# Coder-Yu/QRec

Measured on NVIDIA H100. Metric: BPR triples/sec at d=64, higher is better.
Workload: dtype f32

## Files before the change

### qrec_b200/csrc/bpr_kernels.cu

```cuda
#include <cmath>

#include "common.h"
#include "device.cuh"
#include "philox.cuh"
#include "bpr_step.cuh"

namespace {

using namespace qrec;
using namespace qrec::bpr;

template <typename T, int E>
__global__ void __launch_bounds__(256)
bpr_sgd_ordered_kernel(T* __restrict__ P, T* __restrict__ Q, int d, long long n,
                       const int* __restrict__ u, const int* __restrict__ i,
                       const int* __restrict__ j, const int* __restrict__ wu,
                       const int* __restrict__ wi, const int* __restrict__ wj, int* ver_p,
                       int* ver_q, unsigned long long* ticket, T lr, T reg_u, T reg_i,
                       double* loss) {
  const int lane = threadIdx.x & 31;
  double local_loss = 0.0;
  const T a_u = mul_rn(lr, reg_u), a_i = mul_rn(lr, reg_i);
  while (true) {
    unsigned long long k = 0;
    if (lane == 0) k = atomicAdd(ticket, 1ULL);
    k = __shfl_sync(0xffffffffu, k, 0);
    if (k >= (unsigned long long)n) break;
    const int uu = u[k], ii = i[k], jj = j[k];
    const int* vp = lane == 0 ? ver_p + uu : (lane == 1 ? ver_q + ii : ver_q + jj);
    const int need = lane == 0 ? wu[k] : (lane == 1 ? wi[k] : wj[k]);
    unsigned backoff = 8, polls = 0;
    while (true) {
      const int have = lane < 3 ? ld_acquire_gpu(vp) : need;
      if (__all_sync(0xffffffffu, have == need)) break;
      __nanosleep(backoff);
      if (backoff < 64) backoff <<= 1;
      if (++polls > (1u << 27)) __trap();
    }
    T* pr = P + (size_t)uu * d;
    T* qir = Q + (size_t)ii * d;
    T* qjr = Q + (size_t)jj * d;
    T p[E], qi[E], qj[E];
    T di = 0, dj = 0;
#pragma unroll
    for (int e = 0; e < E; ++e) {
      const int c = e * 32 + lane;
      if (c < d) {
        p[e] = __ldcg(pr + c);
        qi[e] = __ldcg(qir + c);
        qj[e] = __ldcg(qjr + c);
        di += p[e] * qi[e];
        dj += p[e] * qj[e];
      } else {
        p[e] = qi[e] = qj[e] = 0;
      }
    }
    di = warp_sum(di);
    dj = warp_sum(dj);
// ... 187 lines not shown
          p[r] = *reinterpret_cast<const float4*>(P + (size_t)uu[r] * D + l * 4);
          qi[r] = *reinterpret_cast<const float4*>(Q + (size_t)ii[r] * D + l * 4);
          qj[r] = *reinterpret_cast<const float4*>(Q + (size_t)jj[r] * D + l * 4);
        } else {
          p[r] = qi[r] = qj[r] = make_float4(0.f, 0.f, 0.f, 0.f);
        }
      }
      if (l < 3) asm volatile("cp.async.bulk.wait_group.read 1;" ::: "memory");
      __syncwarp();
      float* slot = my_stage + (size_t)buf * SLOT_FLOATS;
#pragma unroll
      for (int r = 0; r < UNROLL; ++r) {
        float x = dot4(p[r], qi[r]) - dot4(p[r], qj[r]);
        x = group_sum<LPR>(x);
        const float s = fast_sigmoid(x);
        const float g = lr * (1.0f - s);
        if (ok[r]) {
          if (l == 0) lsum += fast_neg_log(s);
          float4 dp, dqi, dqj;
          bpr_step4(p[r], qi[r], qj[r], g, a_u, a_i, dp, dqi, dqj);
          float* trip = slot + (size_t)(r * TPW + sub) * ROWS * D;
          if (TMA_MASK & 1) *reinterpret_cast<float4*>(trip + SLOT_P * D + l * 4) = dp;
          else red_add_v4(P + (size_t)uu[r] * D + l * 4, dp);
          if (TMA_MASK & 2) *reinterpret_cast<float4*>(trip + SLOT_I * D + l * 4) = dqi;
          else red_add_v4(Q + (size_t)ii[r] * D + l * 4, dqi);
          if (TMA_MASK & 4) *reinterpret_cast<float4*>(trip + SLOT_J * D + l * 4) = dqj;
          else red_add_v4(Q + (size_t)jj[r] * D + l * 4, dqj);
        }
      }
      asm volatile("fence.proxy.async.shared::cta;" ::: "memory");
      __syncwarp();
      if (l < 3 && ((TMA_MASK >> l) & 1)) {
        const int srow = (l == 0) ? SLOT_P : (l == 1 ? SLOT_I : SLOT_J);
#pragma unroll
        for (int r = 0; r < UNROLL; ++r) {
          if (ok[r]) {
            float* dst = (l == 0) ? (P + (size_t)uu[r] * D) : (Q + (size_t)(l == 1 ? ii[r] : jj[r]) * D);
            const float* src = slot + (size_t)(r * TPW + sub) * ROWS * D + srow * D;
            asm volatile("cp.reduce.async.bulk.global.shared::cta.bulk_group.add.f32 [%0], [%1], %2;" ::"l"(dst),
                         "r"((uint32_t)__cvta_generic_to_shared(src)), "n"(D * 4)
                         : "memory");
          }
        }
        asm volatile("cp.async.bulk.commit_group;" ::: "memory");
      }
      buf ^= 1;
    }
  }
  if (l < 3) asm volatile("cp.async.bulk.wait_group 0;" ::: "memory");
  block_add_loss(lsum, loss);
}


constexpr int UM_CH = 32;
constexpr int UM_STAGE_FLOATS = 2 * 4 * 64;
constexpr int UM_STAGE_GROUPS = 16;
constexpr int UM_STAGE_SMEM = UM_STAGE_GROUPS * 2 * (UM_STAGE_FLOATS * 4 + 8);

__device__ __forceinline__ void bulk_row_load(float* smem_dst, const float* gsrc, uint64_t* bar) {
  asm volatile("cp.async.bulk.shared::cluster.global.mbarrier::complete_tx::bytes [%0], [%1], 256, [%2];"
               ::"r"(smem_u32(smem_dst)), "l"(gsrc), "r"(smem_u32(bar)) : "memory");
}

template <int LPR, int G, int CH, bool FULL, bool SAMPLE, bool SIG, bool TMA>
__device__ __forceinline__ void
usermajor_epoch(float* __restrict__ P, float* __restrict__ Q, const float* __restrict__ Qr, int nvec, int n_users,
                long long n, long long ch_begin, long long ch_end, const long long* __restrict__ rowptr,
                const int* __restrict__ i, const int* __restrict__ j, float lr,
                float reg_u, float reg_i, double* loss, FusedSampler fs, long long trip_off,
                const uint32_t* __restrict__ rated_sig) {
  static_assert(!TMA || (LPR == 16 && G == 4 && FULL), "the TMA fetch is laid out for d = 64, G = 4");
  constexpr int GPW = 32 / LPR;
  const int lane = threadIdx.x & 31;
  const int sub = lane / LPR, l = lane % LPR;
  const unsigned gmask = (LPR == 32) ? 0xffffffffu : (((1u << LPR) - 1u) << (sub * LPR));
  const long long group = (((long long)blockIdx.x * blockDim.x + threadIdx.x) >> 5) * GPW + sub;
  const long long ngroups = (((long long)gridDim.x * blockDim.x) >> 5) * GPW;
  const int d = FULL ? LPR * 4 : nvec * 4;
  const bool act = FULL ? true : (l < nvec);
  const float a_u = lr * reg_u, a_i = lr * reg_i;
  const float one_m_au = 1.0f - a_u, one_m_ai = 1.0f - a_i;
  float lsum = 0.f;
  float* stage = nullptr;
  uint64_t* bar = nullptr;
  uint32_t phase0 = 0, phase1 = 0;
  if constexpr (TMA) {
    extern __shared__ __align__(128) unsigned char smem_raw[];
    float* stage_all = reinterpret_cast<float*>(smem_raw);
    uint64_t* bars = reinterpret_cast<uint64_t*>(stage_all + UM_STAGE_GROUPS * 2 * UM_STAGE_FLOATS);
    const int g_in_cta = (threadIdx.x >> 5) * GPW + sub;
    stage = stage_all + (size_t)g_in_cta * 2 * UM_STAGE_FLOATS;
    bar = bars + g_in_cta * 2;
    if (l == 0) { mbar_init(bar, 1); mbar_init(bar + 1, 1); }
    asm volatile("fence.mbarrier_init.release.cluster;" ::: "memory");
    asm volatile("fence.proxy.async.shared::cta;" ::: "memory");
    __syncthreads();
  }
  auto user_of = [&](long long t) {
    int a = 0, b = n_users - 1;
    while (a < b) {
      const int len = b - a + 1;
      const int step = (len + LPR - 1) / LPR;
      int pp = a + (l + 1) * step - 1;
      if (pp > b) pp = b;
      const bool pred = (__ldg(rowptr + pp + 1) - trip_off) > t;
      const unsigned bal = (__ballot_sync(gmask, pred) & gmask) >> (sub * LPR);
      const int f = __ffs(bal) - 1;
      int pf = a + (f + 1) * step - 1;
      if (pf > b) pf = b;
      a = a + f * step;
      b = pf;
    }
    return a;
  };
  for (long long ch = ch_begin + group; ch < ch_end; ch += ngroups) {
    long long lo = ch * CH;
    long long hi = (lo + CH) < n ? (lo + CH) : n;
    int uu = user_of(lo);
    if (lo > 0 && __ldg(rowptr + uu) - trip_off < lo) {
      lo = __ldg(rowptr + uu + 1) - trip_off;
      ++uu;
    }
    if (hi < n) {
      const int ub = user_of(hi);
      if (__ldg(rowptr + ub) - trip_off < hi) {
        const long long e = __ldg(rowptr + ub + 1) - trip_off;
        hi = e < n ? e : n;
      }
    }
    if (lo >= hi) continue;
    long long uend = __ldg(rowptr + uu + 1) - trip_off;
    float* prow = P + (size_t)uu * d + l * 4;
    float4 p = act ? *reinterpret_cast<const float4*>(prow) : make_float4(0.f, 0.f, 0.f, 0.f);
    float4 p0 = p;
    for (long long base = lo; base < hi; base += LPR) {
      const int m = (hi - base) < LPR ? (int)(hi - base) : LPR;
      int mi = 0, mj = 0;
      if (l < m) {
        mi = __ldg(i + base + l);
        if (SAMPLE) {
          int us = uu;
          long long ue = uend;
          while (ue <= base + l) {
            ++us;
            ue = __ldg(rowptr + us + 1) - trip_off;
          }
          if (SIG)
            mj = qrec::sample_negative_sig(base + l + trip_off, fs.epoch, fs.seed_lo, fs.seed_hi, fs.num_items,
                                           fs.rated_cols, __ldg(fs.rated_rowptr + us), __ldg(fs.rated_rowptr + us + 1),
                                           rated_sig + (size_t)us * qrec::RATED_SIG_WORDS);
          else
            mj = qrec::sample_negative(base + l + trip_off, fs.epoch, fs.seed_lo, fs.seed_hi, fs.num_items, fs.rated_cols,
                                       __ldg(fs.rated_rowptr + us), __ldg(fs.rated_rowptr + us + 1));
          if (fs.j_out != nullptr) fs.j_out[base + l] = mj;
        } else {
          mj = __ldg(j + base + l);
        }
      }
      auto issue = [&](int t0) {
        const int src = sub * LPR + ((t0 + (l >> 1)) & (LPR - 1));
        const int idi = __shfl_sync(gmask, mi, src), idj = __shfl_sync(gmask, mj, src);
        const int rows_now = 2 * ((m - t0) < G ? (m - t0) : G);
        uint64_t* bb = bar + ((t0 / G) & 1);
        if (l == 0) mbar_expect_tx(bb, 256u * rows_now);
        __syncwarp(gmask);
        if (l < rows_now) bulk_row_load(stage + ((t0 / G) & 1) * UM_STAGE_FLOATS + l * 64, Qr + (size_t)((l & 1) ? idj : idi) * d, bb);
      };
      if constexpr (TMA) issue(0);
      for (int t0 = 0; t0 < m; t0 += G) {
        const float* slot = nullptr;
        if constexpr (TMA) {
          if (t0 + G < m) issue(t0 + G);
          const int s = (t0 / G) & 1;
          mbar_wait(bar + s, s ? phase1 : phase0);
          if (s) phase1 ^= 1u; else phase0 ^= 1u;
          slot = stage + s * UM_STAGE_FLOATS;
        }
        float4 qi[G], qj[G];
        int ri[G], rj[G];
#pragma unroll
        for (int f = 0; f < G; ++f) {
          ri[f] = __shfl_sync(gmask, mi, sub * LPR + ((t0 + f) & (LPR - 1)));
          rj[f] = __shfl_sync(gmask, mj, sub * LPR + ((t0 + f) & (LPR - 1)));
          if (t0 + f < m && act) {
            if constexpr (TMA) {
              qi[f] = *reinterpret_cast<const float4*>(slot + (2 * f) * 64 + l * 4);
              qj[f] = *reinterpret_cast<const float4*>(slot + (2 * f + 1) * 64 + l * 4);
            } else {
              qi[f] = __ldg(reinterpret_cast<const float4*>(Qr + (size_t)ri[f] * d + l * 4));
              qj[f] = __ldg(reinterpret_cast<const float4*>(Qr + (size_t)rj[f] * d + l * 4));
            }
          } else {
            qi[f] = qj[f] = make_float4(0.f, 0.f, 0.f, 0.f);
          }
        }
        if constexpr (TMA) __syncwarp(gmask);
#pragma unroll
        for (int f = 0; f < G; ++f) {
          const long long t = base + t0 + f;
          if (t0 + f < m) {
            if (t >= uend) {
              if (act) red_add_v4(prow, make_float4(p.x - p0.x, p.y - p0.y, p.z - p0.z, p.w - p0.w));
              do {
                ++uu;
                uend = __ldg(rowptr + uu + 1) - trip_off;
              } while (uend <= t);
              prow = P + (size_t)uu * d + l * 4;
              p = act ? *reinterpret_cast<const float4*>(prow) : make_float4(0.f, 0.f, 0.f, 0.f);
              p0 = p;
            }
            float x = dot4(p, qi[f]) - dot4(p, qj[f]);
            x = group_sum<LPR>(x, gmask);
            const float s = fast_sigmoid(x);
            const float g = lr * (1.0f - s);
            if (l == 0) lsum += fast_neg_log(s);
            if (act) {
              float4 dqi, dqj;
              bpr_step4_inplace(p, qi[f], qj[f], g, one_m_au, g * one_m_ai, a_i, dqi, dqj);
              red_add_v4(Q + (size_t)ri[f] * d + l * 4, dqi);
              red_add_v4(Q + (size_t)rj[f] * d + l * 4, dqj);
            }
          }
        }
      }
    }
    if (act) red_add_v4(prow, make_float4(p.x - p0.x, p.y - p0.y, p.z - p0.z, p.w - p0.w));
  }
  block_add_loss(lsum, loss);
}

template <int LPR, int G, int CH, bool FULL, bool SAMPLE, int MINB = 3, bool SIG = false>
__global__ void __launch_bounds__(256, MINB)
bpr_sgd_usermajor_kernel(float* __restrict__ P, float* __restrict__ Q, const float* __restrict__ Qr, int nvec, int n_users,
                         long long n, long long ch_begin, long long ch_end, const long long* __restrict__ rowptr,
                         const int* __restrict__ i, const int* __restrict__ j, float lr,
                         float reg_u, float reg_i, double* loss, FusedSampler fs, long long trip_off,
                         const uint32_t* __restrict__ rated_sig) {
  usermajor_epoch<LPR, G, CH, FULL, SAMPLE, SIG, false>(P, Q, Qr, nvec, n_users, n, ch_begin, ch_end, rowptr, i, j, lr,
                                                         reg_u, reg_i, loss, fs, trip_off, rated_sig);
}

__global__ void __launch_bounds__(256, 3)
bpr_sgd_usermajor_tma_kernel(float* __restrict__ P, float* __restrict__ Q, const float* __restrict__ Qr, int nvec,
                             int n_users, long long n, long long ch_begin, long long ch_end,
                             const long long* __restrict__ rowptr, const int* __restrict__ i, const int* __restrict__ j,
                             float lr, float reg_u, float reg_i, double* loss, FusedSampler fs, long long trip_off,
                             const uint32_t* __restrict__ rated_sig) {
  usermajor_epoch<16, 4, UM_CH, true, true, false, true>(P, Q, Qr, nvec, n_users, n, ch_begin, ch_end, rowptr, i, j,
                                                         lr, reg_u, reg_i, loss, fs, trip_off, rated_sig);
}

using UserMajorKernel = decltype(&bpr_sgd_usermajor_tma_kernel);

template <int LPR>
UserMajorKernel usermajor_kernel(int nvec, bool sample, bool sig) {
  if (nvec != LPR)
    return sample ? bpr_sgd_usermajor_kernel<LPR, 4, UM_CH, false, true> : bpr_sgd_usermajor_kernel<LPR, 4, UM_CH, false, false>;
  if (sig) return bpr_sgd_usermajor_kernel<LPR, 4, UM_CH, true, true, 3, true>;
  return sample ? bpr_sgd_usermajor_kernel<LPR, 4, UM_CH, true, true> : bpr_sgd_usermajor_kernel<LPR, 4, UM_CH, true, false>;
}

__global__ void __launch_bounds__(256)
rated_signature_kernel(int n_users, const long long* __restrict__ rowptr, const int* __restrict__ cols,
                       uint32_t* __restrict__ sig) {
  const int lane = threadIdx.x & 31;
  const long long warp = ((long long)blockIdx.x * blockDim.x + threadIdx.x) >> 5;
  const long long nwarps = ((long long)gridDim.x * blockDim.x) >> 5;
  for (long long uu = warp; uu < n_users; uu += nwarps) {
    const long long lo = __ldg(rowptr + uu), hi = __ldg(rowptr + uu + 1);
    for (long long e = lo + lane; e < hi; e += 32) {
      const int c = __ldg(cols + e);
      atomicOr(sig + (size_t)uu * qrec::RATED_SIG_WORDS + ((c >> 5) & (qrec::RATED_SIG_WORDS - 1)), 1u << (c & 31));
    }
  }
}

template <typename T>
__global__ void __launch_bounds__(256)
sumsq_kernel(const T* __restrict__ x, long long n, double* out) {
  double acc = 0.0;
  const long long tid = (long long)blockIdx.x * blockDim.x + threadIdx.x;
  const long long stride = (long long)gridDim.x * blockDim.x;
  if constexpr (sizeof(T) == 4) {
    const long long n4 = n >> 2;
    const float4* x4 = reinterpret_cast<const float4*>(x);
    for (long long k = tid; k < n4; k += stride) {
      const float4 v = __ldg(x4 + k);
      acc += (double)v.x * v.x + (double)v.y * v.y + (double)v.z * v.z + (double)v.w * v.w;
    }
    for (long long k = (n4 << 2) + tid; k < n; k += stride) acc += (double)x[k] * x[k];
  } else {
    for (long long k = tid; k < n; k += stride) acc += (double)x[k] * (double)x[k];
  }
  acc = warp_sum(acc);
  __shared__ double wsum[8];
  if ((threadIdx.x & 31) == 0) wsum[threadIdx.x >> 5] = acc;
  __syncthreads();
  if (threadIdx.x == 0) {
    double t = 0.0;
    for (int w = 0; w < (int)(blockDim.x >> 5); ++w) t += wsum[w];
    atomicAdd(out, t);
  }
}

template <typename T>
int launch_ordered(T* P, T* Q, int d, long long n, const int* u, const int* i, const int* j,
                   const int* wu, const int* wi, const int* wj, int* ver_p, int* ver_q,
                   unsigned long long* ticket, T lr, T reg_u, T reg_i, double* loss,
                   int n_warps, cudaStream_t st) {
  QREC_REQUIRE(P && Q && loss && ticket && ver_p && ver_q, "bpr_sgd_ordered: null pointer");
  QREC_REQUIRE(d >= 1 && d <= 256, "bpr_sgd_ordered: d=%d unsupported (1..256)", d);
  QREC_REQUIRE(n >= 0, "bpr_sgd_ordered: n < 0");
// ... 59 lines not shown
                             double reg_u, double reg_i, double* loss, int32_t n_warps, void* stream) {
  return launch_ordered<double>(P, Q, d, n, u, i, j, wu, wi, wj, ver_p, ver_q, ticket, lr, reg_u,
                                reg_i, loss, n_warps, (cudaStream_t)stream);
}

int qrec_bpr_sgd_batch_f32(float* P, float* Q, int32_t d, int64_t n, const int32_t* u,
                           const int32_t* i, const int32_t* j, float lr, float reg_u,
                           float reg_i, double* loss, void* stream) {
  return qrec::launch_bpr_batch(P, Q, d, n, u, i, j, lr, reg_u, reg_i, loss, (cudaStream_t)stream);
}

int qrec_bpr_sgd_batch_tma_f32(float* P, float* Q, int32_t d, int64_t n, const int32_t* u,
                               const int32_t* i, const int32_t* j, float lr, float reg_u,
                               float reg_i, double* loss, void* stream) {
  QREC_REQUIRE(P && Q && loss, "qrec_bpr_sgd_batch_tma_f32: null pointer");
  QREC_REQUIRE(d == 64, "qrec_bpr_sgd_batch_tma_f32: only d=64 (got %d); use qrec_bpr_sgd_batch_f32", d);
  QREC_REQUIRE(n >= 0, "qrec_bpr_sgd_batch_tma_f32: n < 0");
  if (n == 0) return QREC_OK;
  QREC_REQUIRE(u && i && j, "qrec_bpr_sgd_batch_tma_f32: null index pointer");
  constexpr int UN = 4, MASK = 1;
  constexpr int smem = 8 * 2 * UN * 2 * 64 * 4;
  QREC_CUDA(allow_dynamic_smem((const void*)bpr_sgd_batch_tma_kernel<UN, MASK>, smem));
  const int grid = capped_grid(((n + 31) / 32 + 7) / 8, 2);
  bpr_sgd_batch_tma_kernel<UN, MASK><<<grid, 256, smem, (cudaStream_t)stream>>>(P, Q, n, u, i, j, lr, reg_u, reg_i, loss);
  QREC_LAUNCH_CHECK();
  return QREC_OK;
}

}

namespace qrec {
int launch_usermajor(float* P, float* Q, int32_t d, int32_t n_users, int64_t n, const int64_t* rowptr,
                     const int32_t* i, const int32_t* j, float lr, float reg_u, float reg_i, double* loss,
                     bool sample, const int64_t* rated_rowptr, const int32_t* rated_cols, int32_t num_items,
                     uint64_t seed, uint32_t epoch, int32_t* j_out, long long trip_off, cudaStream_t st,
                     const uint32_t* rated_sig, bool tma) {
  if (n <= 0) return QREC_OK;
  QREC_REQUIRE(num_items >= 1, "qrec user-major epoch: num_items=%d (the item table's rows) must be given", num_items);
  QREC_REQUIRE(!tma || (d == 64 && sample), "qrec user-major epoch: the TMA fetch needs d = 64 and fused sampling");
  FusedSampler fs = {reinterpret_cast<const long long*>(rated_rowptr), rated_cols, num_items, (uint32_t)seed,
                     (uint32_t)(seed >> 32), epoch, j_out};
  const int nvec = d / 4;
  const int lpr = nvec <= 4 ? 4 : nvec <= 8 ? 8 : nvec <= 16 ? 16 : 32;
  const bool sig = sample && rated_sig != nullptr;
  const UserMajorKernel kernel = tma        ? bpr_sgd_usermajor_tma_kernel
                                 : lpr == 4  ? usermajor_kernel<4>(nvec, sample, sig)
                                 : lpr == 8  ? usermajor_kernel<8>(nvec, sample, sig)
                                 : lpr == 16 ? usermajor_kernel<16>(nvec, sample, sig)
                                             : usermajor_kernel<32>(nvec, sample, sig);
  const int smem = tma ? UM_STAGE_SMEM : 0;
  if (tma) QREC_CUDA(allow_dynamic_smem((const void*)kernel, smem));
  int occ = 3;
  if (cudaOccupancyMaxActiveBlocksPerMultiprocessor(&occ, kernel, 256, smem) != cudaSuccess || occ < 1) occ = 3;
  const long long nchunks = (n + UM_CH - 1) / UM_CH;
  const long long per_block = 8 * (32 / lpr);
  const int grid = capped_grid((nchunks + per_block - 1) / per_block, occ);
  const size_t q_bytes = (size_t)num_items * d * sizeof(float);
  const long long copy_bytes = 2 * (long long)q_bytes;
  const long long copy_floor = copy_bytes > (8LL << 20) ? 8 * copy_bytes / (24LL * d + 12) : 0;
  long long wave_triples = n / 64 > copy_floor ? n / 64 : copy_floor;
  if (wave_triples > 4LL * num_items) wave_triples = 4LL * num_items;
  const long long wave = wave_triples / UM_CH > 1 ? wave_triples / UM_CH : 1;
  float* Qr = nullptr;
  QREC_CUDA(cudaMallocAsync(reinterpret_cast<void**>(&Qr), q_bytes, st));
  const int rc = [&]() -> int {
    for (long long c0 = 0; c0 < nchunks; c0 += wave) {
      QREC_CUDA(cudaMemcpyAsync(Qr, Q, q_bytes, cudaMemcpyDeviceToDevice, st));
      const long long c1 = (c0 + wave) < nchunks ? (c0 + wave) : nchunks;
      kernel<<<grid, 256, smem, st>>>(P, Q, Qr, nvec, n_users, n, c0, c1, reinterpret_cast<const long long*>(rowptr), i, j,
                                      lr, reg_u, reg_i, loss, fs, trip_off, rated_sig);
      QREC_CUDA(cudaGetLastError());
      if (c1 < nchunks) count_launch();
    }
    return QREC_OK;
  }();
  QREC_CUDA(cudaFreeAsync(Qr, st));
  if (rc != QREC_OK) return rc;
  QREC_LAUNCH_CHECK();
  return QREC_OK;
}
}

extern "C" {

int qrec_bpr_sgd_usermajor_f32(float* P, float* Q, int32_t d, int32_t n_users, int64_t n, int32_t num_items,
                               const int64_t* rowptr, const int32_t* i, const int32_t* j, float lr, float reg_u, float reg_i,
                               double* loss, void* stream) {
  QREC_REQUIRE(P && Q && loss, "qrec_bpr_sgd_usermajor_f32: null pointer");
  QREC_REQUIRE(d >= 4 && d <= 128 && (d % 4) == 0, "qrec_bpr_sgd_usermajor_f32: d=%d unsupported (multiple of 4, 4..128)", d);
  QREC_REQUIRE(n_users >= 0 && n >= 0, "qrec_bpr_sgd_usermajor_f32: negative size");
  if (n_users == 0 || n == 0) return QREC_OK;
  QREC_REQUIRE(rowptr && i && j, "qrec_bpr_sgd_usermajor_f32: null index pointer");
  return qrec::launch_usermajor(P, Q, d, n_users, n, rowptr, i, j, lr, reg_u, reg_i, loss, false, nullptr, nullptr, num_items,
                                0, 0, nullptr, 0, (cudaStream_t)stream, nullptr, false);
}

int qrec_bpr_epoch_usermajor_f32(float* P, float* Q, int32_t d, int32_t n_users, int64_t n, const int64_t* rowptr,
                                 const int32_t* i, const int64_t* rated_rowptr, const int32_t* rated_cols,
                                 int32_t num_items, uint64_t seed, uint32_t epoch, int32_t* j_out, float lr,
                                 float reg_u, float reg_i, double* loss, void* stream) {
  QREC_REQUIRE(P && Q && loss, "qrec_bpr_epoch_usermajor_f32: null pointer");
  QREC_REQUIRE(d >= 4 && d <= 128 && (d % 4) == 0, "qrec_bpr_epoch_usermajor_f32: d=%d unsupported (multiple of 4, 4..128)", d);
  QREC_REQUIRE(n_users >= 0 && n >= 0 && num_items >= 1, "qrec_bpr_epoch_usermajor_f32: bad size");
  if (n_users == 0 || n == 0) return QREC_OK;
  QREC_REQUIRE(rowptr && i && rated_rowptr && rated_cols, "qrec_bpr_epoch_usermajor_f32: null index pointer");
  return qrec::launch_usermajor(P, Q, d, n_users, n, rowptr, i, nullptr, lr, reg_u, reg_i, loss, true, rated_rowptr,
                                rated_cols, num_items, seed, epoch, j_out, 0, (cudaStream_t)stream, nullptr, false);
}

int qrec_rated_signature_build(int32_t n_users, const int64_t* rated_rowptr, const int32_t* rated_cols,
                               uint32_t* sig, void* stream) {
  QREC_REQUIRE(n_users >= 0, "qrec_rated_signature_build: n_users < 0");
  if (n_users == 0) return QREC_OK;
  QREC_REQUIRE(rated_rowptr && rated_cols && sig, "qrec_rated_signature_build: null pointer");
  cudaStream_t st = (cudaStream_t)stream;
  QREC_CUDA(cudaMemsetAsync(sig, 0, (size_t)n_users * qrec::RATED_SIG_WORDS * sizeof(uint32_t), st));
  rated_signature_kernel<<<capped_grid(((long long)n_users + 7) / 8, 8), 256, 0, st>>>(n_users, reinterpret_cast<const long long*>(rated_rowptr),
                                                     rated_cols, sig);
  QREC_LAUNCH_CHECK();
  return QREC_OK;
}

int qrec_bpr_epoch_usermajor_sig_f32(float* P, float* Q, int32_t d, int32_t n_users, int64_t n, const int64_t* rowptr,
                                     const int32_t* i, const int64_t* rated_rowptr, const int32_t* rated_cols,
                                     const uint32_t* rated_sig, int32_t num_items, uint64_t seed, uint32_t epoch,
                                     int32_t* j_out, float lr, float reg_u, float reg_i, double* loss, void* stream) {
  QREC_REQUIRE(P && Q && loss, "qrec_bpr_epoch_usermajor_sig_f32: null pointer");
  QREC_REQUIRE(d == 16 || d == 32 || d == 64 || d == 128,
// ... 67 lines not shown
```

### qrec_b200/csrc/philox.cuh

```cuda
#pragma once
#include <cstdint>

namespace qrec {

__device__ __forceinline__ void philox4x32_10(uint32_t c0, uint32_t c1, uint32_t c2, uint32_t c3,
                                              uint32_t k0, uint32_t k1, uint32_t out[4]) {
  constexpr uint32_t M0 = 0xD2511F53u, M1 = 0xCD9E8D57u, W0 = 0x9E3779B9u, W1 = 0xBB67AE85u;
#pragma unroll
  for (int r = 0; r < 10; ++r) {
    const uint32_t hi0 = __umulhi(M0, c0), lo0 = M0 * c0;
    const uint32_t hi1 = __umulhi(M1, c2), lo1 = M1 * c2;
    const uint32_t n0 = hi1 ^ c1 ^ k0, n1 = lo1, n2 = hi0 ^ c3 ^ k1, n3 = lo0;
    c0 = n0; c1 = n1; c2 = n2; c3 = n3;
    k0 += W0; k1 += W1;
  }
  out[0] = c0; out[1] = c1; out[2] = c2; out[3] = c3;
}

__device__ __forceinline__ int sample_negative(long long k, uint32_t epoch, uint32_t seed_lo, uint32_t seed_hi,
                                               int num_items, const int* __restrict__ cols, long long lo0,
                                               long long hi0) {
  const bool saturated = (hi0 - lo0) >= (long long)num_items;
  uint32_t attempt = 0;
  while (true) {
    uint32_t w[4];
    philox4x32_10((uint32_t)k, (uint32_t)((unsigned long long)k >> 32), attempt, epoch, seed_lo, seed_hi, w);
    const int j = (int)(((unsigned long long)w[0] * (unsigned long long)(uint32_t)num_items) >> 32);
    if (saturated) return j;
    long long lo = lo0, hi = hi0;
    bool hit = false;
    while (lo < hi) {
      const long long mid = (lo + hi) >> 1;
      const int c = __ldg(cols + mid);
      if (c < j) lo = mid + 1;
      else if (c > j) hi = mid;
      else { hit = true; break; }
    }
    if (!hit) return j;
    ++attempt;
  }
}

constexpr int RATED_SIG_WORDS = 16;
__device__ __forceinline__ int sample_negative_sig(long long k, uint32_t epoch, uint32_t seed_lo, uint32_t seed_hi,
                                                   int num_items, const int* __restrict__ cols, long long lo0,
                                                   long long hi0, const uint32_t* __restrict__ sig) {
  const bool saturated = (hi0 - lo0) >= (long long)num_items;
  uint32_t attempt = 0;
  while (true) {
    uint32_t w[4];
    philox4x32_10((uint32_t)k, (uint32_t)((unsigned long long)k >> 32), attempt, epoch, seed_lo, seed_hi, w);
    const int j = (int)(((unsigned long long)w[0] * (unsigned long long)(uint32_t)num_items) >> 32);
    if (saturated) return j;
    const uint32_t word = __ldg(sig + ((j >> 5) & (RATED_SIG_WORDS - 1)));
    if (((word >> (j & 31)) & 1u) == 0u) return j;
    long long lo = lo0, hi = hi0;
    bool hit = false;
    while (lo < hi) {
      const long long mid = (lo + hi) >> 1;
      const int c = __ldg(cols + mid);
      if (c < j) lo = mid + 1;
      else if (c > j) hi = mid;
      else { hit = true; break; }
    }
    if (!hit) return j;
    ++attempt;
  }
}

struct FusedSampler {
  const long long* rated_rowptr;
  const int* rated_cols;
  int num_items;
  uint32_t seed_lo, seed_hi, epoch;
  int* j_out;
};

}
```

Measured before the change: 2.650 billion.

## Schedule user-major BPR by precomputed per-wave user plan with register-cached rated lists

Replaces chunk-based scheduling (per-chunk warp-cooperative binary search over rowptr plus mid-chunk user switching) with a small plan kernel that binary-searches wave boundaries once. Each group then processes whole users strided across the grid. Per-user rated-item lists (up to 64) and signature words are cached in registers, and negative-sample rejection is done by warp shuffles instead of per-lane global binary search. This cuts index-search and scattered-load overhead, but load balance now depends on user-degree skew, and the all-to-all shuffle check costs many instructions.

After: 2.692 billion, median of 6. +1.6%, better.

```diff
diff --git a/qrec_b200/csrc/bpr_kernels.cu b/qrec_b200/csrc/bpr_kernels.cu
--- a/qrec_b200/csrc/bpr_kernels.cu
+++ b/qrec_b200/csrc/bpr_kernels.cu
@@ -298,6 +298,7 @@
 
 
 constexpr int UM_CH = 32;
+constexpr int UM_RATED_PER_LANE = 4;
 constexpr int UM_STAGE_FLOATS = 2 * 4 * 64;
 constexpr int UM_STAGE_GROUPS = 16;
 constexpr int UM_STAGE_SMEM = UM_STAGE_GROUPS * 2 * (UM_STAGE_FLOATS * 4 + 8);
@@ -307,10 +308,27 @@
                ::"r"(smem_u32(smem_dst)), "l"(gsrc), "r"(smem_u32(bar)) : "memory");
 }
 
-template <int LPR, int G, int CH, bool FULL, bool SAMPLE, bool SIG, bool TMA>
+__global__ void __launch_bounds__(256)
+usermajor_wave_plan_kernel(const long long* __restrict__ rowptr, int n_users, long long trip_off, long long wave_triples,
+                           int n_waves, int* __restrict__ plan) {
+  const int w = blockIdx.x * blockDim.x + threadIdx.x;
+  if (w > n_waves) return;
+  if (w == n_waves) { plan[w] = n_users; return; }
+  const long long t = (long long)w * wave_triples;
+  int a = 0, b = n_users;
+  while (a < b) {
+    const int mid = (a + b) >> 1;
+    const long long s = __ldg(rowptr + mid) - trip_off;
+    if ((s > 0 ? s : 0) >= t) b = mid;
+    else a = mid + 1;
+  }
+  plan[w] = a;
+}
+
+template <int LPR, int G, bool FULL, bool SAMPLE, bool SIG, bool TMA>
 __device__ __forceinline__ void
-usermajor_epoch(float* __restrict__ P, float* __restrict__ Q, const float* __restrict__ Qr, int nvec, int n_users,
-                long long n, long long ch_begin, long long ch_end, const long long* __restrict__ rowptr,
+usermajor_epoch(float* __restrict__ P, float* __restrict__ Q, const float* __restrict__ Qr, int nvec, long long n,
+                const int* __restrict__ plan, int wave, const long long* __restrict__ rowptr,
                 const int* __restrict__ i, const int* __restrict__ j, float lr,
                 float reg_u, float reg_i, double* loss, FusedSampler fs, long long trip_off,
                 const uint32_t* __restrict__ rated_sig) {
@@ -319,8 +337,8 @@
   const int lane = threadIdx.x & 31;
   const int sub = lane / LPR, l = lane % LPR;
   const unsigned gmask = (LPR == 32) ? 0xffffffffu : (((1u << LPR) - 1u) << (sub * LPR));
-  const long long group = (((long long)blockIdx.x * blockDim.x + threadIdx.x) >> 5) * GPW + sub;
-  const long long ngroups = (((long long)gridDim.x * blockDim.x) >> 5) * GPW;
+  const int g_in_cta = (threadIdx.x >> 5) * GPW + sub;
+  const int ngroups = gridDim.x * (int)(blockDim.x / LPR);
   const int d = FULL ? LPR * 4 : nvec * 4;
   const bool act = FULL ? true : (l < nvec);
   const float a_u = lr * reg_u, a_i = lr * reg_i;
@@ -333,7 +351,6 @@
     extern __shared__ __align__(128) unsigned char smem_raw[];
     float* stage_all = reinterpret_cast<float*>(smem_raw);
     uint64_t* bars = reinterpret_cast<uint64_t*>(stage_all + UM_STAGE_GROUPS * 2 * UM_STAGE_FLOATS);
-    const int g_in_cta = (threadIdx.x >> 5) * GPW + sub;
     stage = stage_all + (size_t)g_in_cta * 2 * UM_STAGE_FLOATS;
     bar = bars + g_in_cta * 2;
     if (l == 0) { mbar_init(bar, 1); mbar_init(bar + 1, 1); }
@@ -341,66 +358,72 @@
     asm volatile("fence.proxy.async.shared::cta;" ::: "memory");
     __syncthreads();
   }
-  auto user_of = [&](long long t) {
-    int a = 0, b = n_users - 1;
-    while (a < b) {
-      const int len = b - a + 1;
-      const int step = (len + LPR - 1) / LPR;
-      int pp = a + (l + 1) * step - 1;
-      if (pp > b) pp = b;
-      const bool pred = (__ldg(rowptr + pp + 1) - trip_off) > t;
-      const unsigned bal = (__ballot_sync(gmask, pred) & gmask) >> (sub * LPR);
-      const int f = __ffs(bal) - 1;
-      int pf = a + (f + 1) * step - 1;
-      if (pf > b) pf = b;
-      a = a + f * step;
-      b = pf;
-    }
-    return a;
-  };
-  for (long long ch = ch_begin + group; ch < ch_end; ch += ngroups) {
-    long long lo = ch * CH;
-    long long hi = (lo + CH) < n ? (lo + CH) : n;
-    int uu = user_of(lo);
-    if (lo > 0 && __ldg(rowptr + uu) - trip_off < lo) {
-      lo = __ldg(rowptr + uu + 1) - trip_off;
-      ++uu;
-    }
-    if (hi < n) {
-      const int ub = user_of(hi);
-      if (__ldg(rowptr + ub) - trip_off < hi) {
-        const long long e = __ldg(rowptr + ub + 1) - trip_off;
-        hi = e < n ? e : n;
-      }
-    }
-    if (lo >= hi) continue;
-    long long uend = __ldg(rowptr + uu + 1) - trip_off;
+  const int u_end = __ldg(plan + wave + 1);
+  for (int uu = __ldg(plan + wave) + g_in_cta * (int)gridDim.x + blockIdx.x; uu < u_end; uu += ngroups) {
+    long long s = __ldg(rowptr + uu) - trip_off, e = __ldg(rowptr + uu + 1) - trip_off;
+    const long long rlo = SAMPLE ? __ldg(fs.rated_rowptr + uu) : 0, rhi = SAMPLE ? __ldg(fs.rated_rowptr + uu + 1) : 0;
+    s = s > 0 ? s : 0;
+    e = e < n ? e : n;
+    if (s >= e) continue;
+    constexpr int SW = (qrec::RATED_SIG_WORDS + LPR - 1) / LPR;
+    const long long rcnt = rhi - rlo;
+    const bool saturated = rcnt >= (long long)fs.num_items;
+    const bool row_in_regs = rcnt <= UM_RATED_PER_LANE * LPR;
+    int rc[UM_RATED_PER_LANE];
+    uint32_t sw[SW];
+#pragma unroll
+    for (int v = 0; v < UM_RATED_PER_LANE; ++v)
+      rc[v] = (SAMPLE && row_in_regs && l + v * LPR < rcnt) ? __ldg(fs.rated_cols + rlo + l + v * LPR) : -1;
+#pragma unroll
+    for (int w = 0; w < SW; ++w)
+      sw[w] = (SIG && l + w * LPR < qrec::RATED_SIG_WORDS) ? __ldg(rated_sig + (size_t)uu * qrec::RATED_SIG_WORDS + l + w * LPR) : 0u;
     float* prow = P + (size_t)uu * d + l * 4;
     float4 p = act ? *reinterpret_cast<const float4*>(prow) : make_float4(0.f, 0.f, 0.f, 0.f);
-    float4 p0 = p;
-    for (long long base = lo; base < hi; base += LPR) {
-      const int m = (hi - base) < LPR ? (int)(hi - base) : LPR;
+    const float4 p0 = p;
+    for (long long base = s; base < e; base += LPR) {
+      const int m = (e - base) < LPR ? (int)(e - base) : LPR;
       int mi = 0, mj = 0;
-      if (l < m) {
-        mi = __ldg(i + base + l);
-        if (SAMPLE) {
-          int us = uu;
-          long long ue = uend;
-          while (ue <= base + l) {
-            ++us;
-            ue = __ldg(rowptr + us + 1) - trip_off;
+      if (l < m) mi = __ldg(i + base + l);
+      if constexpr (SAMPLE) {
+        const long long k = base + l + trip_off;
+        bool drawing = l < m;
+        for (uint32_t attempt = 0; __any_sync(gmask, drawing); ++attempt) {
+          const int jj = drawing ? qrec::negative_draw(k, attempt, fs.epoch, fs.seed_lo, fs.seed_hi, fs.num_items) : -1;
+          bool maybe = drawing && !saturated;
+          if constexpr (SIG) {
+            const int wd = (jj >> 5) & (qrec::RATED_SIG_WORDS - 1);
+            uint32_t word = 0;
+#pragma unroll
+            for (int w = 0; w < SW; ++w) {
+              const uint32_t t = __shfl_sync(gmask, sw[w], sub * LPR + (wd % LPR));
+              if (w == wd / LPR) word = t;
+            }
+            maybe = maybe && ((word >> (jj & 31)) & 1u);
           }
-          if (SIG)
-            mj = qrec::sample_negative_sig(base + l + trip_off, fs.epoch, fs.seed_lo, fs.seed_hi, fs.num_items,
-                                           fs.rated_cols, __ldg(fs.rated_rowptr + us), __ldg(fs.rated_rowptr + us + 1),
-                                           rated_sig + (size_t)us * qrec::RATED_SIG_WORDS);
-          else
-            mj = qrec::sample_negative(base + l + trip_off, fs.epoch, fs.seed_lo, fs.seed_hi, fs.num_items, fs.rated_cols,
-                                       __ldg(fs.rated_rowptr + us), __ldg(fs.rated_rowptr + us + 1));
-          if (fs.j_out != nullptr) fs.j_out[base + l] = mj;
-        } else {
-          mj = __ldg(j + base + l);
+          bool rated = false;
+          if (row_in_regs) {
+            if (__any_sync(gmask, maybe)) {
+#pragma unroll
+              for (int src = 0; src < LPR; ++src)
+#pragma unroll
+                for (int v = 0; v < UM_RATED_PER_LANE; ++v) rated |= __shfl_sync(gmask, rc[v], sub * LPR + src) == jj;
+              rated = rated && maybe;
+            }
+          } else if (maybe) {
+            long long lo = rlo, hi = rhi;
+            while (lo < hi && !rated) {
+              const long long mid = (lo + hi) >> 1;
+              const int c = __ldg(fs.rated_cols + mid);
+              if (c < jj) lo = mid + 1;
+              else if (c > jj) hi = mid;
+              else rated = true;
+            }
+          }
+          if (drawing && !rated) { mj = jj; drawing = false; }
         }
+        if (l < m && fs.j_out != nullptr) fs.j_out[base + l] = mj;
+      } else {
+        if (l < m) mj = __ldg(j + base + l);
       }
       auto issue = [&](int t0) {
         const int src = sub * LPR + ((t0 + (l >> 1)) & (LPR - 1));
@@ -413,13 +436,13 @@
       };
       if constexpr (TMA) issue(0);
       for (int t0 = 0; t0 < m; t0 += G) {
-        const float* slot = nullptr;
+        const float* rows = nullptr;
         if constexpr (TMA) {
           if (t0 + G < m) issue(t0 + G);
-          const int s = (t0 / G) & 1;
-          mbar_wait(bar + s, s ? phase1 : phase0);
-          if (s) phase1 ^= 1u; else phase0 ^= 1u;
-          slot = stage + s * UM_STAGE_FLOATS;
+          const int sl = (t0 / G) & 1;
+          mbar_wait(bar + sl, sl ? phase1 : phase0);
+          if (sl) phase1 ^= 1u; else phase0 ^= 1u;
+          rows = stage + sl * UM_STAGE_FLOATS;
         }
         float4 qi[G], qj[G];
         int ri[G], rj[G];
@@ -429,8 +452,8 @@
           rj[f] = __shfl_sync(gmask, mj, sub * LPR + ((t0 + f) & (LPR - 1)));
           if (t0 + f < m && act) {
             if constexpr (TMA) {
-              qi[f] = *reinterpret_cast<const float4*>(slot + (2 * f) * 64 + l * 4);
-              qj[f] = *reinterpret_cast<const float4*>(slot + (2 * f + 1) * 64 + l * 4);
+              qi[f] = *reinterpret_cast<const float4*>(rows + (2 * f) * 64 + l * 4);
+              qj[f] = *reinterpret_cast<const float4*>(rows + (2 * f + 1) * 64 + l * 4);
             } else {
               qi[f] = __ldg(reinterpret_cast<const float4*>(Qr + (size_t)ri[f] * d + l * 4));
               qj[f] = __ldg(reinterpret_cast<const float4*>(Qr + (size_t)rj[f] * d + l * 4));
@@ -442,23 +465,12 @@
         if constexpr (TMA) __syncwarp(gmask);
 #pragma unroll
         for (int f = 0; f < G; ++f) {
-          const long long t = base + t0 + f;
           if (t0 + f < m) {
-            if (t >= uend) {
-              if (act) red_add_v4(prow, make_float4(p.x - p0.x, p.y - p0.y, p.z - p0.z, p.w - p0.w));
-              do {
-                ++uu;
-                uend = __ldg(rowptr + uu + 1) - trip_off;
-              } while (uend <= t);
-              prow = P + (size_t)uu * d + l * 4;
-              p = act ? *reinterpret_cast<const float4*>(prow) : make_float4(0.f, 0.f, 0.f, 0.f);
-              p0 = p;
-            }
             float x = dot4(p, qi[f]) - dot4(p, qj[f]);
             x = group_sum<LPR>(x, gmask);
-            const float s = fast_sigmoid(x);
-            const float g = lr * (1.0f - s);
-            if (l == 0) lsum += fast_neg_log(s);
+            const float sg = fast_sigmoid(x);
+            const float g = lr * (1.0f - sg);
+            if (l == 0) lsum += fast_neg_log(sg);
             if (act) {
               float4 dqi, dqj;
               bpr_step4_inplace(p, qi[f], qj[f], g, one_m_au, g * one_m_ai, a_i, dqi, dqj);
@@ -476,23 +488,22 @@
 
 template <int LPR, int G, int CH, bool FULL, bool SAMPLE, int MINB = 3, bool SIG = false>
 __global__ void __launch_bounds__(256, MINB)
-bpr_sgd_usermajor_kernel(float* __restrict__ P, float* __restrict__ Q, const float* __restrict__ Qr, int nvec, int n_users,
-                         long long n, long long ch_begin, long long ch_end, const long long* __restrict__ rowptr,
+bpr_sgd_usermajor_kernel(float* __restrict__ P, float* __restrict__ Q, const float* __restrict__ Qr, int nvec, long long n,
+                         const int* __restrict__ plan, int wave, const long long* __restrict__ rowptr,
                          const int* __restrict__ i, const int* __restrict__ j, float lr,
                          float reg_u, float reg_i, double* loss, FusedSampler fs, long long trip_off,
                          const uint32_t* __restrict__ rated_sig) {
-  usermajor_epoch<LPR, G, CH, FULL, SAMPLE, SIG, false>(P, Q, Qr, nvec, n_users, n, ch_begin, ch_end, rowptr, i, j, lr,
-                                                         reg_u, reg_i, loss, fs, trip_off, rated_sig);
+  usermajor_epoch<LPR, G, FULL, SAMPLE, SIG, false>(P, Q, Qr, nvec, n, plan, wave, rowptr, i, j, lr, reg_u, reg_i, loss, fs,
+                                                    trip_off, rated_sig);
 }
 
 __global__ void __launch_bounds__(256, 3)
 bpr_sgd_usermajor_tma_kernel(float* __restrict__ P, float* __restrict__ Q, const float* __restrict__ Qr, int nvec,
-                             int n_users, long long n, long long ch_begin, long long ch_end,
-                             const long long* __restrict__ rowptr, const int* __restrict__ i, const int* __restrict__ j,
-                             float lr, float reg_u, float reg_i, double* loss, FusedSampler fs, long long trip_off,
-                             const uint32_t* __restrict__ rated_sig) {
-  usermajor_epoch<16, 4, UM_CH, true, true, false, true>(P, Q, Qr, nvec, n_users, n, ch_begin, ch_end, rowptr, i, j,
-                                                         lr, reg_u, reg_i, loss, fs, trip_off, rated_sig);
+                             long long n, const int* __restrict__ plan, int wave, const long long* __restrict__ rowptr,
+                             const int* __restrict__ i, const int* __restrict__ j, float lr, float reg_u, float reg_i,
+                             double* loss, FusedSampler fs, long long trip_off, const uint32_t* __restrict__ rated_sig) {
+  usermajor_epoch<16, 4, true, true, false, true>(P, Q, Qr, nvec, n, plan, wave, rowptr, i, j, lr, reg_u, reg_i, loss, fs,
+                                                  trip_off, rated_sig);
 }
 
 using UserMajorKernel = decltype(&bpr_sgd_usermajor_tma_kernel);
@@ -677,19 +688,25 @@
   long long wave_triples = n / 64 > copy_floor ? n / 64 : copy_floor;
   if (wave_triples > 4LL * num_items) wave_triples = 4LL * num_items;
   const long long wave = wave_triples / UM_CH > 1 ? wave_triples / UM_CH : 1;
+  const int n_waves = (int)((nchunks + wave - 1) / wave);
+  const long long* rp = reinterpret_cast<const long long*>(rowptr);
   float* Qr = nullptr;
+  int* plan = nullptr;
   QREC_CUDA(cudaMallocAsync(reinterpret_cast<void**>(&Qr), q_bytes, st));
+  QREC_CUDA(cudaMallocAsync(reinterpret_cast<void**>(&plan), sizeof(int) * (size_t)(n_waves + 1), st));
   const int rc = [&]() -> int {
-    for (long long c0 = 0; c0 < nchunks; c0 += wave) {
+    usermajor_wave_plan_kernel<<<(n_waves + 256) / 256, 256, 0, st>>>(rp, n_users, trip_off, wave * UM_CH, n_waves, plan);
+    QREC_CUDA(cudaGetLastError());
+    count_launch();
+    for (int w = 0; w < n_waves; ++w) {
       QREC_CUDA(cudaMemcpyAsync(Qr, Q, q_bytes, cudaMemcpyDeviceToDevice, st));
-      const long long c1 = (c0 + wave) < nchunks ? (c0 + wave) : nchunks;
-      kernel<<<grid, 256, smem, st>>>(P, Q, Qr, nvec, n_users, n, c0, c1, reinterpret_cast<const long long*>(rowptr), i, j,
-                                      lr, reg_u, reg_i, loss, fs, trip_off, rated_sig);
+      kernel<<<grid, 256, smem, st>>>(P, Q, Qr, nvec, n, plan, w, rp, i, j, lr, reg_u, reg_i, loss, fs, trip_off, rated_sig);
       QREC_CUDA(cudaGetLastError());
-      if (c1 < nchunks) count_launch();
+      if (w + 1 < n_waves) count_launch();
     }
     return QREC_OK;
   }();
+  QREC_CUDA(cudaFreeAsync(plan, st));
   QREC_CUDA(cudaFreeAsync(Qr, st));
   if (rc != QREC_OK) return rc;
   QREC_LAUNCH_CHECK();
diff --git a/qrec_b200/csrc/philox.cuh b/qrec_b200/csrc/philox.cuh
--- a/qrec_b200/csrc/philox.cuh
+++ b/qrec_b200/csrc/philox.cuh
@@ -17,15 +17,20 @@
   out[0] = c0; out[1] = c1; out[2] = c2; out[3] = c3;
 }
 
+__device__ __forceinline__ int negative_draw(long long k, uint32_t attempt, uint32_t epoch, uint32_t seed_lo,
+                                             uint32_t seed_hi, int num_items) {
+  uint32_t w[4];
+  philox4x32_10((uint32_t)k, (uint32_t)((unsigned long long)k >> 32), attempt, epoch, seed_lo, seed_hi, w);
+  return (int)(((unsigned long long)w[0] * (unsigned long long)(uint32_t)num_items) >> 32);
+}
+
 __device__ __forceinline__ int sample_negative(long long k, uint32_t epoch, uint32_t seed_lo, uint32_t seed_hi,
                                                int num_items, const int* __restrict__ cols, long long lo0,
                                                long long hi0) {
   const bool saturated = (hi0 - lo0) >= (long long)num_items;
   uint32_t attempt = 0;
   while (true) {
-    uint32_t w[4];
-    philox4x32_10((uint32_t)k, (uint32_t)((unsigned long long)k >> 32), attempt, epoch, seed_lo, seed_hi, w);
-    const int j = (int)(((unsigned long long)w[0] * (unsigned long long)(uint32_t)num_items) >> 32);
+    const int j = negative_draw(k, attempt, epoch, seed_lo, seed_hi, num_items);
     if (saturated) return j;
     long long lo = lo0, hi = hi0;
     bool hit = false;
@@ -48,9 +53,7 @@
   const bool saturated = (hi0 - lo0) >= (long long)num_items;
   uint32_t attempt = 0;
   while (true) {
-    uint32_t w[4];
-    philox4x32_10((uint32_t)k, (uint32_t)((unsigned long long)k >> 32), attempt, epoch, seed_lo, seed_hi, w);
-    const int j = (int)(((unsigned long long)w[0] * (unsigned long long)(uint32_t)num_items) >> 32);
+    const int j = negative_draw(k, attempt, epoch, seed_lo, seed_hi, num_items);
     if (saturated) return j;
     const uint32_t word = __ldg(sig + ((j >> 5) & (RATED_SIG_WORDS - 1)));
     if (((word >> (j & 31)) & 1u) == 0u) return j;
```

## Assign whole users to warp groups via precomputed per-wave user ranges

Applied to the files above, without the earlier changes.

Replaces chunk-based scheduling, which needed per-chunk binary searches over rowptr and mid-chunk user switches, with one user per group. Each wave's user range comes from a small table computed on the device. The rated-item row bounds are now loaded once per user, and the per-triple user walk in the sampler is removed. The P delta is now formed by re-reading the row with __ldcg at the end. This adds a table kernel and allocation and can cause load imbalance for users with many interactions. The sampled full-width kernels also change G from 4 to 2 and min-blocks from 3 to 4.

Measured after the change: 2.576 billion before, 2.802 billion after, median of 6. 8.8% higher.

```diff
diff --git a/qrec_b200/csrc/bpr_kernels.cu b/qrec_b200/csrc/bpr_kernels.cu
--- a/qrec_b200/csrc/bpr_kernels.cu
+++ b/qrec_b200/csrc/bpr_kernels.cu
@@ -4,6 +4,7 @@
 #include "device.cuh"
 #include "philox.cuh"
 #include "bpr_step.cuh"
+#include "um_waves.cuh"
 
 namespace {
 
@@ -297,7 +298,6 @@
 }
 
 
-constexpr int UM_CH = 32;
 constexpr int UM_STAGE_FLOATS = 2 * 4 * 64;
 constexpr int UM_STAGE_GROUPS = 16;
 constexpr int UM_STAGE_SMEM = UM_STAGE_GROUPS * 2 * (UM_STAGE_FLOATS * 4 + 8);
@@ -307,20 +307,19 @@
                ::"r"(smem_u32(smem_dst)), "l"(gsrc), "r"(smem_u32(bar)) : "memory");
 }
 
-template <int LPR, int G, int CH, bool FULL, bool SAMPLE, bool SIG, bool TMA>
+template <int LPR, int G, bool FULL, bool SAMPLE, bool SIG, bool TMA>
 __device__ __forceinline__ void
-usermajor_epoch(float* __restrict__ P, float* __restrict__ Q, const float* __restrict__ Qr, int nvec, int n_users,
-                long long n, long long ch_begin, long long ch_end, const long long* __restrict__ rowptr,
-                const int* __restrict__ i, const int* __restrict__ j, float lr,
-                float reg_u, float reg_i, double* loss, FusedSampler fs, long long trip_off,
-                const uint32_t* __restrict__ rated_sig) {
+usermajor_epoch(float* __restrict__ P, float* __restrict__ Q, const float* __restrict__ Qr, int nvec, long long n,
+                const int* __restrict__ wave_user, const long long* __restrict__ rowptr, const int* __restrict__ i,
+                const int* __restrict__ j, float lr, float reg_u, float reg_i, double* loss, FusedSampler fs,
+                long long trip_off, const uint32_t* __restrict__ rated_sig) {
   static_assert(!TMA || (LPR == 16 && G == 4 && FULL), "the TMA fetch is laid out for d = 64, G = 4");
   constexpr int GPW = 32 / LPR;
   const int lane = threadIdx.x & 31;
   const int sub = lane / LPR, l = lane % LPR;
   const unsigned gmask = (LPR == 32) ? 0xffffffffu : (((1u << LPR) - 1u) << (sub * LPR));
-  const long long group = (((long long)blockIdx.x * blockDim.x + threadIdx.x) >> 5) * GPW + sub;
-  const long long ngroups = (((long long)gridDim.x * blockDim.x) >> 5) * GPW;
+  const int group = (int)((blockIdx.x * blockDim.x + threadIdx.x) >> 5) * GPW + sub;
+  const int ngroups = (int)((gridDim.x * blockDim.x) >> 5) * GPW;
   const int d = FULL ? LPR * 4 : nvec * 4;
   const bool act = FULL ? true : (l < nvec);
   const float a_u = lr * reg_u, a_i = lr * reg_i;
@@ -341,62 +340,32 @@
     asm volatile("fence.proxy.async.shared::cta;" ::: "memory");
     __syncthreads();
   }
-  auto user_of = [&](long long t) {
-    int a = 0, b = n_users - 1;
-    while (a < b) {
-      const int len = b - a + 1;
-      const int step = (len + LPR - 1) / LPR;
-      int pp = a + (l + 1) * step - 1;
-      if (pp > b) pp = b;
-      const bool pred = (__ldg(rowptr + pp + 1) - trip_off) > t;
-      const unsigned bal = (__ballot_sync(gmask, pred) & gmask) >> (sub * LPR);
-      const int f = __ffs(bal) - 1;
-      int pf = a + (f + 1) * step - 1;
-      if (pf > b) pf = b;
-      a = a + f * step;
-      b = pf;
-    }
-    return a;
-  };
-  for (long long ch = ch_begin + group; ch < ch_end; ch += ngroups) {
-    long long lo = ch * CH;
-    long long hi = (lo + CH) < n ? (lo + CH) : n;
-    int uu = user_of(lo);
-    if (lo > 0 && __ldg(rowptr + uu) - trip_off < lo) {
-      lo = __ldg(rowptr + uu + 1) - trip_off;
-      ++uu;
-    }
-    if (hi < n) {
-      const int ub = user_of(hi);
-      if (__ldg(rowptr + ub) - trip_off < hi) {
-        const long long e = __ldg(rowptr + ub + 1) - trip_off;
-        hi = e < n ? e : n;
-      }
-    }
+  const int ub = __ldg(wave_user + 1);
+  for (int uu = __ldg(wave_user) + group; uu < ub; uu += ngroups) {
+    long long lo = __ldg(rowptr + uu) - trip_off, hi = __ldg(rowptr + uu + 1) - trip_off;
+    lo = lo > 0 ? lo : 0;
+    hi = hi < n ? hi : n;
     if (lo >= hi) continue;
-    long long uend = __ldg(rowptr + uu + 1) - trip_off;
     float* prow = P + (size_t)uu * d + l * 4;
     float4 p = act ? *reinterpret_cast<const float4*>(prow) : make_float4(0.f, 0.f, 0.f, 0.f);
-    float4 p0 = p;
+    long long rated_lo = 0, rated_hi = 0;
+    if (SAMPLE) {
+      rated_lo = __ldg(fs.rated_rowptr + uu);
+      rated_hi = __ldg(fs.rated_rowptr + uu + 1);
+    }
     for (long long base = lo; base < hi; base += LPR) {
       const int m = (hi - base) < LPR ? (int)(hi - base) : LPR;
       int mi = 0, mj = 0;
       if (l < m) {
         mi = __ldg(i + base + l);
         if (SAMPLE) {
-          int us = uu;
-          long long ue = uend;
-          while (ue <= base + l) {
-            ++us;
-            ue = __ldg(rowptr + us + 1) - trip_off;
-          }
           if (SIG)
             mj = qrec::sample_negative_sig(base + l + trip_off, fs.epoch, fs.seed_lo, fs.seed_hi, fs.num_items,
-                                           fs.rated_cols, __ldg(fs.rated_rowptr + us), __ldg(fs.rated_rowptr + us + 1),
-                                           rated_sig + (size_t)us * qrec::RATED_SIG_WORDS);
+                                           fs.rated_cols, rated_lo, rated_hi,
+                                           rated_sig + (size_t)uu * qrec::RATED_SIG_WORDS);
           else
             mj = qrec::sample_negative(base + l + trip_off, fs.epoch, fs.seed_lo, fs.seed_hi, fs.num_items, fs.rated_cols,
-                                       __ldg(fs.rated_rowptr + us), __ldg(fs.rated_rowptr + us + 1));
+                                       rated_lo, rated_hi);
           if (fs.j_out != nullptr) fs.j_out[base + l] = mj;
         } else {
           mj = __ldg(j + base + l);
@@ -442,18 +411,7 @@
         if constexpr (TMA) __syncwarp(gmask);
 #pragma unroll
         for (int f = 0; f < G; ++f) {
-          const long long t = base + t0 + f;
           if (t0 + f < m) {
-            if (t >= uend) {
-              if (act) red_add_v4(prow, make_float4(p.x - p0.x, p.y - p0.y, p.z - p0.z, p.w - p0.w));
-              do {
-                ++uu;
-                uend = __ldg(rowptr + uu + 1) - trip_off;
-              } while (uend <= t);
-              prow = P + (size_t)uu * d + l * 4;
-              p = act ? *reinterpret_cast<const float4*>(prow) : make_float4(0.f, 0.f, 0.f, 0.f);
-              p0 = p;
-            }
             float x = dot4(p, qi[f]) - dot4(p, qj[f]);
             x = group_sum<LPR>(x, gmask);
             const float s = fast_sigmoid(x);
@@ -469,30 +427,31 @@
         }
       }
     }
-    if (act) red_add_v4(prow, make_float4(p.x - p0.x, p.y - p0.y, p.z - p0.z, p.w - p0.w));
+    if (act) {
+      const float4 p0 = __ldcg(reinterpret_cast<const float4*>(prow));
+      red_add_v4(prow, make_float4(p.x - p0.x, p.y - p0.y, p.z - p0.z, p.w - p0.w));
+    }
   }
   block_add_loss(lsum, loss);
 }
 
-template <int LPR, int G, int CH, bool FULL, bool SAMPLE, int MINB = 3, bool SIG = false>
+template <int LPR, int G, bool FULL, bool SAMPLE, int MINB = 3, bool SIG = false>
 __global__ void __launch_bounds__(256, MINB)
-bpr_sgd_usermajor_kernel(float* __restrict__ P, float* __restrict__ Q, const float* __restrict__ Qr, int nvec, int n_users,
-                         long long n, long long ch_begin, long long ch_end, const long long* __restrict__ rowptr,
-                         const int* __restrict__ i, const int* __restrict__ j, float lr,
-                         float reg_u, float reg_i, double* loss, FusedSampler fs, long long trip_off,
-                         const uint32_t* __restrict__ rated_sig) {
-  usermajor_epoch<LPR, G, CH, FULL, SAMPLE, SIG, false>(P, Q, Qr, nvec, n_users, n, ch_begin, ch_end, rowptr, i, j, lr,
-                                                         reg_u, reg_i, loss, fs, trip_off, rated_sig);
+bpr_sgd_usermajor_kernel(float* __restrict__ P, float* __restrict__ Q, const float* __restrict__ Qr, int nvec, long long n,
+                         const int* __restrict__ wave_user, const long long* __restrict__ rowptr,
+                         const int* __restrict__ i, const int* __restrict__ j, float lr, float reg_u, float reg_i,
+                         double* loss, FusedSampler fs, long long trip_off, const uint32_t* __restrict__ rated_sig) {
+  usermajor_epoch<LPR, G, FULL, SAMPLE, SIG, false>(P, Q, Qr, nvec, n, wave_user, rowptr, i, j, lr, reg_u, reg_i, loss, fs,
+                                                    trip_off, rated_sig);
 }
 
 __global__ void __launch_bounds__(256, 3)
 bpr_sgd_usermajor_tma_kernel(float* __restrict__ P, float* __restrict__ Q, const float* __restrict__ Qr, int nvec,
-                             int n_users, long long n, long long ch_begin, long long ch_end,
-                             const long long* __restrict__ rowptr, const int* __restrict__ i, const int* __restrict__ j,
-                             float lr, float reg_u, float reg_i, double* loss, FusedSampler fs, long long trip_off,
-                             const uint32_t* __restrict__ rated_sig) {
-  usermajor_epoch<16, 4, UM_CH, true, true, false, true>(P, Q, Qr, nvec, n_users, n, ch_begin, ch_end, rowptr, i, j,
-                                                         lr, reg_u, reg_i, loss, fs, trip_off, rated_sig);
+                             long long n, const int* __restrict__ wave_user, const long long* __restrict__ rowptr,
+                             const int* __restrict__ i, const int* __restrict__ j, float lr, float reg_u, float reg_i,
+                             double* loss, FusedSampler fs, long long trip_off, const uint32_t* __restrict__ rated_sig) {
+  usermajor_epoch<16, 4, true, true, false, true>(P, Q, Qr, nvec, n, wave_user, rowptr, i, j, lr, reg_u, reg_i, loss, fs,
+                                                  trip_off, rated_sig);
 }
 
 using UserMajorKernel = decltype(&bpr_sgd_usermajor_tma_kernel);
@@ -500,9 +459,16 @@
 template <int LPR>
 UserMajorKernel usermajor_kernel(int nvec, bool sample, bool sig) {
   if (nvec != LPR)
-    return sample ? bpr_sgd_usermajor_kernel<LPR, 4, UM_CH, false, true> : bpr_sgd_usermajor_kernel<LPR, 4, UM_CH, false, false>;
-  if (sig) return bpr_sgd_usermajor_kernel<LPR, 4, UM_CH, true, true, 3, true>;
-  return sample ? bpr_sgd_usermajor_kernel<LPR, 4, UM_CH, true, true> : bpr_sgd_usermajor_kernel<LPR, 4, UM_CH, true, false>;
+    return sample ? bpr_sgd_usermajor_kernel<LPR, 4, false, true> : bpr_sgd_usermajor_kernel<LPR, 4, false, false>;
+  if (sig) return bpr_sgd_usermajor_kernel<LPR, 2, true, true, 4, true>;
+  return sample ? bpr_sgd_usermajor_kernel<LPR, 2, true, true, 4> : bpr_sgd_usermajor_kernel<LPR, 4, true, false>;
+}
+
+__global__ void __launch_bounds__(256)
+um_wave_table_kernel(const long long* __restrict__ rowptr, int n_users, long long n, long long trip_off,
+                     long long wave_chunks, long long nwaves, int* __restrict__ wave_user) {
+  const long long w = (long long)blockIdx.x * blockDim.x + threadIdx.x;
+  if (w <= nwaves) wave_user[w] = um_wave_first_user(rowptr, n_users, n, trip_off, wave_chunks, w);
 }
 
 __global__ void __launch_bounds__(256)
@@ -668,28 +634,31 @@
   if (tma) QREC_CUDA(allow_dynamic_smem((const void*)kernel, smem));
   int occ = 3;
   if (cudaOccupancyMaxActiveBlocksPerMultiprocessor(&occ, kernel, 256, smem) != cudaSuccess || occ < 1) occ = 3;
-  const long long nchunks = (n + UM_CH - 1) / UM_CH;
   const long long per_block = 8 * (32 / lpr);
-  const int grid = capped_grid((nchunks + per_block - 1) / per_block, occ);
+  const long long max_users = n < n_users ? n : n_users;
+  const int grid = capped_grid((max_users + per_block - 1) / per_block, occ);
   const size_t q_bytes = (size_t)num_items * d * sizeof(float);
-  const long long copy_bytes = 2 * (long long)q_bytes;
-  const long long copy_floor = copy_bytes > (8LL << 20) ? 8 * copy_bytes / (24LL * d + 12) : 0;
-  long long wave_triples = n / 64 > copy_floor ? n / 64 : copy_floor;
-  if (wave_triples > 4LL * num_items) wave_triples = 4LL * num_items;
-  const long long wave = wave_triples / UM_CH > 1 ? wave_triples / UM_CH : 1;
+  const long long wave = um_wave_chunks(n, num_items, d);
+  const long long nwaves = um_num_waves(n, wave);
   float* Qr = nullptr;
+  int* wave_user = nullptr;
   QREC_CUDA(cudaMallocAsync(reinterpret_cast<void**>(&Qr), q_bytes, st));
   const int rc = [&]() -> int {
-    for (long long c0 = 0; c0 < nchunks; c0 += wave) {
+    QREC_CUDA(cudaMallocAsync(reinterpret_cast<void**>(&wave_user), sizeof(int) * (size_t)(nwaves + 1), st));
+    um_wave_table_kernel<<<(unsigned)((nwaves + 256) / 256), 256, 0, st>>>(reinterpret_cast<const long long*>(rowptr), n_users,
+                                                                          n, trip_off, wave, nwaves, wave_user);
+    QREC_CUDA(cudaGetLastError());
+    count_launch();
+    for (long long w = 0; w < nwaves; ++w) {
       QREC_CUDA(cudaMemcpyAsync(Qr, Q, q_bytes, cudaMemcpyDeviceToDevice, st));
-      const long long c1 = (c0 + wave) < nchunks ? (c0 + wave) : nchunks;
-      kernel<<<grid, 256, smem, st>>>(P, Q, Qr, nvec, n_users, n, c0, c1, reinterpret_cast<const long long*>(rowptr), i, j,
-                                      lr, reg_u, reg_i, loss, fs, trip_off, rated_sig);
+      kernel<<<grid, 256, smem, st>>>(P, Q, Qr, nvec, n, wave_user + w, reinterpret_cast<const long long*>(rowptr), i, j, lr,
+                                      reg_u, reg_i, loss, fs, trip_off, rated_sig);
       QREC_CUDA(cudaGetLastError());
-      if (c1 < nchunks) count_launch();
+      if (w + 1 < nwaves) count_launch();
     }
     return QREC_OK;
   }();
+  if (wave_user != nullptr) QREC_CUDA(cudaFreeAsync(wave_user, st));
   QREC_CUDA(cudaFreeAsync(Qr, st));
   if (rc != QREC_OK) return rc;
   QREC_LAUNCH_CHECK();
diff --git a/qrec_b200/csrc/um_waves.cuh b/qrec_b200/csrc/um_waves.cuh
--- /dev/null
+++ b/qrec_b200/csrc/um_waves.cuh
@@ -0,0 +1,41 @@
+#pragma once
+
+#if defined(__CUDACC__)
+#define QREC_HD __host__ __device__
+#else
+#define QREC_HD
+#endif
+
+namespace qrec {
+
+constexpr int UM_CH = 32;
+
+QREC_HD inline long long um_wave_chunks(long long n, long long num_items, int d) {
+  const long long copy_bytes = 2 * num_items * d * 4;
+  const long long copy_floor = copy_bytes > (8LL << 20) ? 8 * copy_bytes / (24LL * d + 12) : 0;
+  long long wave_triples = n / 64 > copy_floor ? n / 64 : copy_floor;
+  if (wave_triples > 4 * num_items) wave_triples = 4 * num_items;
+  return wave_triples / UM_CH > 1 ? wave_triples / UM_CH : 1;
+}
+
+QREC_HD inline long long um_num_waves(long long n, long long wave_chunks) {
+  const long long nchunks = (n + UM_CH - 1) / UM_CH;
+  return (nchunks + wave_chunks - 1) / wave_chunks;
+}
+
+QREC_HD inline int um_wave_first_user(const long long* rowptr, int n_users, long long n, long long trip_off,
+                                      long long wave_chunks, long long w) {
+  long long b = w * wave_chunks * UM_CH;
+  if (b > n) b = n;
+  const long long key = b == 0 ? trip_off + 1 : trip_off + b;
+  const long long* a = b == 0 ? rowptr + 1 : rowptr;
+  int lo = 0, hi = b == 0 ? n_users : n_users + 1;
+  while (lo < hi) {
+    const int mid = lo + (hi - lo) / 2;
+    if (a[mid] >= key) hi = mid;
+    else lo = mid + 1;
+  }
+  return lo;
+}
+
+}
```
